# Nikhil-Kulkarni/RayTrace-miniapp

Hardware: AMD Instinct MI355X
Metric: ray_steps_per_sec (higher is better)
Workload: dtype f32+f64

## Files before the change

raytrace-miniapp_amd/csrc/rt_march.hip:

```cpp
#pragma once
#include "rt_math.h"

#include <cfloat>

namespace rt {

enum : int { ST_DONE_ESC = -2, ST_DONE = -1, ST_IDLE = 0, ST_STEP = 1, ST_XSETUP = 2, ST_CELL = 3, ST_ESC = 4 };
static_assert(ST_CELL + ST_DONE - ST_CELL == ST_DONE && ST_CELL + ST_DONE - ST_ESC == ST_DONE_ESC && ST_DONE_ESC < ST_IDLE &&
                  ST_DONE < ST_IDLE && ST_ESC > ST_CELL && ST_CELL > ST_XSETUP && ST_CELL > ST_STEP,
              "the order of the lane states");

typedef double f64x2 __attribute__((ext_vector_type(2)));
typedef float f32x4 __attribute__((ext_vector_type(4)));
typedef unsigned u32x4 __attribute__((ext_vector_type(4)));

__device__ __forceinline__ unsigned div_magic(unsigned x, unsigned mul, unsigned sh)
{
    return mul ? __umulhi(x, mul) >> sh : x;
}
__device__ __forceinline__ void grid_index(const DevRays &R, unsigned ridx, unsigned &i, unsigned &j, unsigned &k,
                                           unsigned &m)
{
    const unsigned ijkm = (unsigned) (R.first + (long long) ridx * R.stride);
    const unsigned q1   = div_magic(ijkm, R.div_mul[0], R.div_sh[0]);
    m                   = ijkm - q1 * (unsigned) R.ngb;
    const unsigned q2   = div_magic(q1, R.div_mul[1], R.div_sh[1]);
    k                   = q1 - q2 * (unsigned) R.nga;
    i                   = div_magic(q2, R.div_mul[2], R.div_sh[2]);
    j                   = q2 - i * (unsigned) R.ngy;
}

__device__ __forceinline__ void load_ray(const DevRays &R, unsigned ridx, rt_ray &ray, float &ta, float &tb,
                                         bool want_tan)
{
    if (R.list) {
        ray = R.list[ridx];
        if (want_tan) {
            ta = R.sxy[2 * (size_t) ridx];
            tb = R.sxy[2 * (size_t) ridx + 1];
        }
    } else {
        unsigned i, j, k, m;
        grid_index(R, ridx, i, j, k, m);
        ray.x      = (float) R.gx[i];
        ray.y      = (float) R.gy[j];
        ray.a      = (float) R.ga[k];
        ray.b      = (float) R.gb[m];
        if (want_tan) {
            ta = R.tan_a[k];
            tb = R.tan_b[m];
        }
    }
}

__device__ __attribute__((noinline)) float tan_wide(float x)
{
    if (!(fabsf(x) <= FLT_MAX))
        return x - x;
    return (float) tan((double) x);
}
__device__ __attribute__((noinline)) float atan_wide(float x)
{
    const float A0 = 3.3333334327e-01f, A1 = -2.0000000298e-01f, A2 = 1.4285714924e-01f, A3 = -1.1111110449e-01f,
                A4 = 9.0908870101e-02f, A5 = -7.6918758452e-02f, A6 = 6.6610731184e-02f, A7 = -5.8335702866e-02f,
                A8 = 4.9768779427e-02f, A9 = -3.6531571299e-02f, A10 = 1.6285819933e-02f;
    const unsigned hx = __float_as_uint(x), ix = hx & 0x7fffffffu;
    const bool neg = (hx >> 31) != 0u;
    if (ix >= 0x4c000000u) {
        if (ix > 0x7f800000u)
            return x + x;
        const float r = 1.5707962513e+00f + 7.5497894159e-08f;
        return neg ? -r : r;
    }
    float hi, lo;
    x = fabsf(x);
    if (ix < 0x3f980000u) {
        if (ix < 0x3f300000u) {
            hi = 4.6364760399e-01f;
            lo = 5.0121582440e-09f;
            x  = (2.0f * x - 1.0f) / (2.0f + x);
        } else {
            hi = 7.8539812565e-01f;
            lo = 3.7748947079e-08f;
            x  = (x - 1.0f) / (x + 1.0f);
        }
    } else {
        if (ix < 0x401c0000u) {
            hi = 9.8279368877e-01f;
            lo = 3.4473217170e-08f;
            x  = (x - 1.5f) / (1.0f + 1.5f * x);
        } else {
            hi = 1.5707962513e+00f;
            lo = 7.5497894159e-08f;
            x  = -1.0f / x;
        }
    }
    const float z = x * x, w = z * z;
    const float s1 = z * (A0 + w * (A2 + w * (A4 + w * (A6 + w * (A8 + w * A10)))));
    const float s2 = w * (A1 + w * (A3 + w * (A5 + w * (A7 + w * A9))));
    const float r  = hi - ((x * (s1 + s2) - lo) - x);
    return neg ? -r : r;
}

__device__ __attribute__((noinline)) float ktanf_flt32(float x, float y, int iy)
{
    const float T[13] = { 3.3333334327e-01f, 1.3333334029e-01f, 5.3968254477e-02f, 2.1869488060e-02f, 8.8632395491e-03f,
                          3.5920790397e-03f, 1.4562094584e-03f, 5.8804126456e-04f, 2.4646313977e-04f, 7.8179444245e-05f,
                          7.1407252108e-05f, -1.8558637748e-05f, 2.5907305826e-05f };
    const float pio4 = 7.8539812565e-01f, pio4lo = 3.7748947079e-08f;
    float z, r, v, w, s;
    const int hx = (int) __float_as_uint(x), ix = hx & 0x7fffffff;
    if (ix < 0x39000000) {
        if ((int) x == 0) {
            if ((ix | (iy + 1)) == 0)
                return 1.0f / fabsf(x);
            else if (iy == 1)
                return x;
            else
                return -1.0f / x;
        }
    }
    if (ix >= 0x3f2ca140) {
        if (hx < 0) {
            x = -x;
            y = -y;
        }
        z = pio4 - x;
        w = pio4lo - y;
        x = z + w;
        y = 0.0f;
        if (fabsf(x) < 0x1p-13f)
            return (1 - ((hx >> 30) & 2)) * iy * (1.0f - 2 * iy * x);
    }
    z = x * x;
    w = z * z;
    r = T[1] + w * (T[3] + w * (T[5] + w * (T[7] + w * (T[9] + w * T[11]))));
    v = z * (T[2] + w * (T[4] + w * (T[6] + w * (T[8] + w * (T[10] + w * T[12])))));
    s = z * x;
    r = y + z * (s * (r + v) + y);
    r += T[0] * s;
    w = x + r;
    if (ix >= 0x3f2ca140) {
        v = (float) iy;
        return (float) (1 - ((hx >> 30) & 2)) * (v - 2.0f * (x - (w * w / (w + v) - r)));
    }
    if (iy == 1)
        return w;
    float a, t;
    z = __uint_as_float(__float_as_uint(w) & 0xfffff000u);
    v = r - (z - x);
    t = a = -1.0f / w;
    t = __uint_as_float(__float_as_uint(t) & 0xfffff000u);
    s = 1.0f + t * z;
    return t + a * (s + t * v);
}
__device__ __attribute__((noinline)) float tanf_flt32_wide(float x)
{
    const float pio2_1 = 1.5707855225e+00f, pio2_1t = 1.0804334124e-05f, pio2_2 = 1.0804273188e-05f,
                pio2_2t = 6.0770999344e-11f;
    const int hx = (int) __float_as_uint(x), ix = hx & 0x7fffffff;
    if (ix <= 0x3f490fda)
        return ktanf_flt32(x, 0.0f, 1);
    float y0, y1, z;
    if (hx > 0) {
        z = x - pio2_1;
        if ((ix & 0xfffffff0) != 0x3fc90fd0) {
            y0 = z - pio2_1t;
            y1 = (z - y0) - pio2_1t;
        } else {
            z -= pio2_2;
            y0 = z - pio2_2t;
            y1 = (z - y0) - pio2_2t;
        }
    } else {
        z = x + pio2_1;
        if ((ix & 0xfffffff0) != 0x3fc90fd0) {
            y0 = z + pio2_1t;
            y1 = (z - y0) + pio2_1t;
        } else {
            z += pio2_2;
            y0 = z + pio2_2t;
            y1 = (z - y0) + pio2_2t;
        }
    }
    return ktanf_flt32(y0, y1, -1);
}

__device__ __forceinline__ float tanf_flt32_kernel(float x)
{
    const float ax = fabsf(x);
    if (ax < 0x1p-13f)
        return x;
    if (ax > 0.2f) {
        if (!(ax <= FLT_MAX))
            return x - x;
        return ax <= 1.375f ? tanf_flt32_wide(x) : tan_wide(x);
    }
    const float T0 = 3.3333334327e-01f, T1 = 1.3333334029e-01f, T2 = 5.3968254477e-02f, T3 = 2.1869488060e-02f,
                T4 = 8.8632395491e-03f, T5 = 3.5920790397e-03f, T6 = 1.4562094584e-03f, T7 = 5.8804126456e-04f,
                T8 = 2.4646313977e-04f, T9 = 7.8179444245e-05f, T10 = 7.1407252108e-05f, T11 = -1.8558637748e-05f,
                T12 = 2.5907305826e-05f;
    const float z = x * x;
    const float w = z * z;
    float r       = T1 + w * (T3 + w * (T5 + w * (T7 + w * (T9 + w * T11))));
    const float v = z * (T2 + w * (T4 + w * (T6 + w * (T8 + w * (T10 + w * T12)))));
    const float s = z * x;
    r             = 0.0f + z * (s * (r + v) + 0.0f);
    r += T0 * s;
    return x + r;
}

__device__ __forceinline__ float atanf_flt32_kernel(float x)
{
    const float ax = fabsf(x);
    if (ax < 0x1p-29f)
        return x;
    if (!(ax < 0.4375f))
        return atan_wide(x);
    const float A0 = 3.3333334327e-01f, A1 = -2.0000000298e-01f, A2 = 1.4285714924e-01f, A3 = -1.1111110449e-01f,
                A4 = 9.0908870101e-02f, A5 = -7.6918758452e-02f, A6 = 6.6610731184e-02f, A7 = -5.8335702866e-02f,
                A8 = 4.9768779427e-02f, A9 = -3.6531571299e-02f, A10 = 1.6285819933e-02f;
    const float z  = x * x;
    const float w  = z * z;
    const float s1 = z * (A0 + w * (A2 + w * (A4 + w * (A6 + w * (A8 + w * A10)))));
    const float s2 = w * (A1 + w * (A3 + w * (A5 + w * (A7 + w * A9))));
    return x - x * (s1 + s2);
}

extern "C" __global__ void __launch_bounds__(256) rt_seed_tab_kernel(const DevSeed sd, const DevRays R, double *sf,
                                                                     unsigned char *sin)
{
    const int n0 = R.ngx, n1 = R.ngy, n2 = R.nga, n3 = R.ngb;
    for (int t = (int) (blockIdx.x * blockDim.x + threadIdx.x); t < n0 + n1 + n2 + n3; t += (int) (gridDim.x * blockDim.x)) {
        int d           = t < n0 ? 0 : (t < n0 + n1 ? 1 : (t < n0 + n1 + n2 ? 2 : 3));
        const int i     = t - (d > 0 ? n0 : 0) - (d > 1 ? n1 : 0) - (d > 2 ? n2 : 0);
        const double *g = d == 0 ? R.gx : (d == 1 ? R.gy : (d == 2 ? R.ga : R.gb));
        const double v  = (double) (float) g[i];
        const bool in   = v >= sd.x[d][0] && v <= sd.x[d][sd.dim[d] - 1];
        sin[t]          = in ? 1 : 0;
        sf[t]           = in ? pchip_eval(sd.dim[d], sd.x[d], sd.f[d], v) : 0.0;
    }
}

__device__ __forceinline__ unsigned selftest_hash(unsigned x)
{
    x ^= x >> 16;
    x *= 0x7feb352du;
    x ^= x >> 15;
    x *= 0x846ca68bu;
    x ^= x >> 16;
    return x;
}
extern "C" __global__ void __launch_bounds__(256) rt_selftest_kernel(unsigned long long *counts)
{
    const unsigned lo = 0x3f700000u, hi = 0x3f880000u;
    const unsigned n_fast = hi - lo, n_other = 1u << 24;
    unsigned long long checked = 0, bad = 0;
    const unsigned long long tid = (unsigned long long) blockIdx.x * blockDim.x + threadIdx.x;
    const unsigned long long nth = (unsigned long long) gridDim.x * blockDim.x;
    for (unsigned long long t = tid; t < (unsigned long long) n_fast + n_other; t += nth) {
        const unsigned u = t < n_fast ? lo + (unsigned) t : (unsigned) (t - n_fast) << 8;
        float q          = __uint_as_float(u);
        const float a    = inv_norm(q);
        asm volatile("" : "+v"(q));
        const float b = 1.0f / sqrtf(q);
        checked++;
        if (__float_as_uint(a) != __float_as_uint(b) && !(a != a && b != b))
            bad++;
    }
    for (unsigned long long t = tid; t < (4ull << 23); t += nth) {
        float n       = __uint_as_float(0x3e800000u + (unsigned) t);
        const float a = fdiv_one_nr(n);
        asm volatile("" : "+v"(n));
        const float b = 1.0f / n;
        checked++;
        bad += __float_as_uint(a) != __float_as_uint(b) ? 1 : 0;
    }
    for (unsigned long long t = tid; t < (1ull << 28); t += nth) {
        const unsigned h0 = selftest_hash((unsigned) t * 2u + 1u), h1 = selftest_hash((unsigned) t * 2u + 0x9e3779b9u);
        const int ea = -84 + (int) (h0 % 84u), eb = -78 + (int) (h1 % 122u);
        if (ea - eb >= 96 || eb - ea >= 96 || ea - eb < -120)
            continue;
        float x = __uint_as_float(((unsigned) (ea + 127) << 23) | (selftest_hash(h0) & 0x7fffffu));
        float y = __uint_as_float(((unsigned) (eb + 127) << 23) | (selftest_hash(h1) & 0x7fffffu));
        const float a = fdiv_nr(x, y);
        asm volatile("" : "+v"(x), "+v"(y));
        const float b = x / y;
        checked++;
        bad += __float_as_uint(a) != __float_as_uint(b) ? 1 : 0;
    }
    if (tid == 0) {
        float inf = __uint_as_float(0x7f800000u), qnan = __uint_as_float(0x7fc00000u), big = 3.0e38f;
        asm volatile("" : "+v"(inf), "+v"(qnan), "+v"(big));
        const unsigned pio2 = 0x3fc90fdbu;
        const float t0 = tanf_flt32_kernel(inf), t1 = tanf_flt32_kernel(-inf), t2 = tanf_flt32_kernel(qnan), t3 = tan_wide(inf),
                    t4 = tan_wide(qnan), t5 = tanf_flt32_kernel(big);
        const float a0 = atanf_flt32_kernel(inf), a1 = atanf_flt32_kernel(-inf), a2 = atanf_flt32_kernel(qnan),
                    a3 = atanf_flt32_kernel(big), a4 = atanf_flt32_kernel(-big);
        checked += 11;
        bad += (t0 == t0) + (t1 == t1) + (t2 == t2) + (t3 == t3) + (t4 == t4) + (__float_as_uint(t5) == 0x7fc12345u);
        bad += (__float_as_uint(a0) != pio2) + (__float_as_uint(a1) != (pio2 | 0x80000000u)) + (a2 == a2) +
               (__float_as_uint(a3) != pio2) + (__float_as_uint(a4) != (pio2 | 0x80000000u));
    }
    atomicAdd(&counts[0], checked);
    atomicAdd(&counts[1], bad);
}

extern "C" __global__ void __launch_bounds__(256) rt_tan_kernel(const rt_ray *rays, unsigned long long n, float *sxy)
{
    unsigned long long i = (unsigned long long) blockIdx.x * blockDim.x + threadIdx.x;
    if (i < n) {
        rt_ray r       = rays[i];
        sxy[2 * i]     = tanf_flt32_kernel(1e-3f * r.a);
        sxy[2 * i + 1] = tanf_flt32_kernel(1e-3f * r.b);
    }
}

__device__ __forceinline__ int bisect_interval(const Interval *iv, int n, double v)
{
    int lo = 0, hi = n - 1;
    while (hi - lo != 1) {
        int mid = (hi + lo) / 2;
        if (iv[mid].hi >= v)
            hi = mid;
        else
            lo = mid;
    }
    return hi;
}
__device__ __forceinline__ int guess_interval(int n, float g0, float inv_h, float v)
{
    return (int) fminf(fmaxf((v - g0) * inv_h, 0.0f), (float) (n - 2)) + 1;
}

#ifdef RT_INSTRUMENT
__device__ unsigned long long g_inst[8];
__device__ unsigned long long g_prune[4];
__device__ unsigned short g_ray_iters[1u << 23];
#endif
#ifdef RT_TIMEBLOCKS
__device__ unsigned long long g_inst[8];
__device__ unsigned long long g_retire[4];
#endif
#ifdef RT_WAVETIMES
__device__ unsigned long long g_wt[8];
__device__ unsigned long long g_wt_end[8192], g_wt_dry[8192];
constexpr int WT_TRACE = 64;
__device__ unsigned long long g_wt_trace[8192][WT_TRACE];
__device__ unsigned g_wt_blocks[8192][WT_TRACE][6];
__device__ unsigned long long g_wt_pub[8192][4];
__device__ unsigned long long g_wt_vm[8192];
#endif
#if defined(RT_INSTRUMENT) || defined(RT_TIMEBLOCKS) || defined(RT_WAVETIMES)
struct MarchDiag {
    static __device__ __forceinline__ unsigned wave_number() { return blockIdx.x * (blockDim.x >> 6) + (threadIdx.x >> 6); }
    static __device__ __forceinline__ bool first_active_lane()
    {
        return (int) (threadIdx.x & 63) == __ffsll((long long) __ballot(1)) - 1;
    }
#ifdef RT_INSTRUMENT
    unsigned w[3] = { 0, 0, 0 }, a[3] = { 0, 0, 0 }, ray_iters = 0;
#endif
#if defined(RT_TIMEBLOCKS) || defined(RT_WAVEBLOCKS)
    unsigned long long tb_acc[6] = { 0, 0, 0, 0, 0, 0 }, tb_last = __builtin_readcyclecounter(), tb_iters = 0;
#endif
#ifdef RT_TIMEBLOCKS
    unsigned rt_fin = 0, rt_blk = 0, rt_refill = 0, rt_dry = 0;
#endif
#ifdef RT_WAVETIMES
    const unsigned long long wt_start = __builtin_amdgcn_s_memrealtime();
    unsigned long long wt_dry = 0, pub_t0 = 0;
    unsigned wt_a_runs = 0, wt_b_runs = 0, wave_iter = 0;
#endif
    __device__ __forceinline__ void tick(int i)
    {
#ifdef RT_INSTRUMENT
        a[i]++;
        w[i] += first_active_lane() ? 1u : 0u;
#endif
    }
    __device__ __forceinline__ void mark(int i)
    {
#if defined(RT_TIMEBLOCKS) || defined(RT_WAVEBLOCKS)
        const unsigned long long now = __builtin_readcyclecounter();
        tb_acc[i] += now - tb_last;
        tb_last = now;
#endif
    }
    __device__ __forceinline__ void iteration(int st, int lane, int n_idle)
    {
#ifdef RT_INSTRUMENT
        ray_iters += st > ST_IDLE ? 1u : 0u;
#endif
#ifdef RT_TIMEBLOCKS
        tb_iters++;
#endif
#ifdef RT_WAVETIMES
        if ((++wave_iter & 15u) == 0u) {
            const unsigned wid = wave_number(), smp = wave_iter >> 4;
            if (lane == 0 && wid < 8192u && smp < (unsigned) WT_TRACE) {
                g_wt_trace[wid][smp] = (__builtin_amdgcn_s_memrealtime() & 0xffffffffffull) | ((unsigned long long) (WAVE - n_idle) << 40) |
                                       ((unsigned long long) wt_a_runs << 48) | ((unsigned long long) wt_b_runs << 56);
                g_wt_trace[wid][0] = smp;
#ifdef RT_WAVEBLOCKS
                for (int b = 0; b < 6; b++)
                    g_wt_blocks[wid][smp][b] = (unsigned) tb_acc[b];
#endif
            }
#ifdef RT_WAVEBLOCKS
            for (int b = 0; b < 6; b++)
                tb_acc[b] = 0;
#endif
            wt_a_runs = wt_b_runs = 0;
        }
#endif
    }
    __device__ __forceinline__ void counters_dry()
    {
#ifdef RT_WAVETIMES
        wt_dry = __builtin_amdgcn_s_memrealtime();
#endif
    }
    __device__ __forceinline__ void blocks_run(bool a_runs, bool lane_wants_b)
    {
#ifdef RT_WAVETIMES
        wt_a_runs += a_runs ? 1u : 0u;
        wt_b_runs += __ballot(lane_wants_b) != 0ull ? 1u : 0u;
#endif
    }
    __device__ __forceinline__ void finishing(int st)
    {
#ifdef RT_TIMEBLOCKS
        rt_fin += (__ballot(st < ST_IDLE) != 0ull && first_active_lane()) ? 1u : 0u;
#endif
    }
    __device__ __forceinline__ void retire_block(int st, bool more)
    {
#ifdef RT_TIMEBLOCKS
        rt_blk += __ballot(st < ST_IDLE) != 0ull ? 1u : 0u;
        rt_dry += more ? 0u : 1u;
#endif
    }
    __device__ __forceinline__ void refill()
    {
#ifdef RT_TIMEBLOCKS
        rt_refill++;
#endif
    }
    __device__ __forceinline__ void ray_retired(unsigned ridx)
    {
#ifdef RT_INSTRUMENT
        if (ridx < (1u << 23))
            g_ray_iters[ridx] = (unsigned short) (ray_iters < 65535u ? ray_iters : 65535u);
        ray_iters = 0;
#endif
    }
    __device__ __forceinline__ void publish_begin()
    {
#ifdef RT_WAVETIMES
        pub_t0 = __builtin_amdgcn_s_memrealtime();
#endif
    }
    __device__ __forceinline__ void publish_stores_landed()
    {
#ifdef RT_WAVETIMES
        const unsigned long long now = __builtin_amdgcn_s_memrealtime();
        atomicAdd(&g_wt_vm[wave_number() & 8191u], now - pub_t0);
        pub_t0 = now;
#endif
    }
    __device__ __forceinline__ void publish_end()
    {
#ifdef RT_WAVETIMES
        const unsigned long long dt = __builtin_amdgcn_s_memrealtime() - pub_t0;
        unsigned long long *q       = g_wt_pub[wave_number() & 8191u];
        atomicAdd(&q[0], dt);
        atomicAdd(&q[1], 1ull);
        atomicMax(&q[3], dt);
#endif
    }
    static __device__ __forceinline__ void push_retry()
    {
#ifdef RT_WAVETIMES
        atomicAdd(&g_wt_pub[wave_number() & 8191u][2], 1ull);
#endif
    }
    __device__ __forceinline__ void tiny_dividend()
    {
#ifdef RT_INSTRUMENT
        if (first_active_lane())
            atomicAdd(&g_inst[6], 1ull);
#endif
    }
    __device__ __forceinline__ void prune(int i)
    {
#ifdef RT_INSTRUMENT
        if (first_active_lane())
            atomicAdd(&g_prune[i], 1ull);
#endif
    }
    __device__ __forceinline__ void wave_end(int lane)
    {
#ifdef RT_WAVETIMES
        if (lane == 0) {
            const unsigned long long wt_end = __builtin_amdgcn_s_memrealtime();
            atomicMin(&g_wt[0], wt_start);
            atomicMax(&g_wt[1], wt_start);
            const unsigned n = atomicAdd((unsigned *) &g_wt[6], 1u);
            if (n < 8192)
                g_wt_end[n] = wt_end | ((unsigned long long) (threadIdx.x >> 6) << 56), g_wt_dry[n] = wt_dry;
        }
#endif
#ifdef RT_TIMEBLOCKS
        const unsigned fin_wave = wave_sum_u32(rt_fin);
        if (lane == 0) {
            for (int i = 0; i < 6; i++)
                atomicAdd(&g_inst[i], tb_acc[i]);
            atomicAdd(&g_inst[7], tb_iters);
            atomicAdd(&g_retire[0], (unsigned long long) fin_wave);
            atomicAdd(&g_retire[1], (unsigned long long) rt_blk);
            atomicAdd(&g_retire[2], (unsigned long long) rt_refill);
            atomicAdd(&g_retire[3], (unsigned long long) rt_dry);
        }
#endif
#ifdef RT_INSTRUMENT
        for (int i = 0; i < 3; i++) {
            const unsigned tw = wave_sum_u32(w[i]), ta = wave_sum_u32(a[i]);
            if (lane == 0) {
                atomicAdd(&g_inst[2 * i], (unsigned long long) tw);
                atomicAdd(&g_inst[2 * i + 1], (unsigned long long) ta);
            }
        }
#endif
    }
};
#else
struct MarchDiag {
    __device__ __forceinline__ void tick(int) {}
    __device__ __forceinline__ void mark(int) {}
    __device__ __forceinline__ void iteration(int, int, int) {}
    __device__ __forceinline__ void counters_dry() {}
    __device__ __forceinline__ void blocks_run(bool, bool) {}
    __device__ __forceinline__ void finishing(int) {}
    __device__ __forceinline__ void retire_block(int, bool) {}
    __device__ __forceinline__ void refill() {}
    __device__ __forceinline__ void ray_retired(unsigned) {}
    __device__ __forceinline__ void publish_begin() {}
    __device__ __forceinline__ void publish_stores_landed() {}
    __device__ __forceinline__ void publish_end() {}
    static __device__ __forceinline__ void push_retry() {}
    __device__ __forceinline__ void tiny_dividend() {}
    __device__ __forceinline__ void prune(int) {}
    __device__ __forceinline__ void wave_end(int) {}
};
#endif

struct TileList {
    unsigned *head;
    unsigned *next;
    unsigned *lnode;
    unsigned *nalloc;
    unsigned cap;
    unsigned *rem;
    unsigned *marching;
    unsigned n_waves;
    unsigned split;
    unsigned k_part;
};
constexpr unsigned TILE_NONE = 0xffffffffu;
constexpr unsigned TILE_PART_FLAG = 1u << 30, TILE_PART_SHIFT = 28, TILE_ID_MASK = (1u << TILE_PART_SHIFT) - 1u;
__device__ __forceinline__ unsigned tile_node(unsigned entry)
{
    return (entry & TILE_ID_MASK) * 4u + ((entry & TILE_PART_FLAG) ? (entry >> TILE_PART_SHIFT) & 3u : 0u);
}
constexpr unsigned TILE_REF_GLOBAL = 1u << 31;
__device__ __forceinline__ void tile_push(const TileList &T, unsigned tile)
{
    const unsigned id = __hip_atomic_fetch_add(T.nalloc, 1u, __ATOMIC_RELAXED, __HIP_MEMORY_SCOPE_WORKGROUP);
    unsigned old      = __hip_atomic_load(T.head, __ATOMIC_RELAXED, __HIP_MEMORY_SCOPE_WORKGROUP);
    if (id < T.cap) {
        __hip_atomic_store(&T.lnode[2u * id], tile, __ATOMIC_RELAXED, __HIP_MEMORY_SCOPE_WORKGROUP);
        for (;;) {
            __hip_atomic_store(&T.lnode[2u * id + 1u], old, __ATOMIC_RELAXED, __HIP_MEMORY_SCOPE_WORKGROUP);
            asm volatile("s_waitcnt lgkmcnt(0)" ::: "memory");
            if (__hip_atomic_compare_exchange_strong(T.head, &old, id, __ATOMIC_RELAXED, __ATOMIC_RELAXED, __HIP_MEMORY_SCOPE_WORKGROUP))
                return;
            MarchDiag::push_retry();
        }
    }
    tile |= TILE_REF_GLOBAL;
    for (;;) {
        __hip_atomic_store(&T.next[tile_node(tile & ~TILE_REF_GLOBAL)], old, __ATOMIC_RELAXED, __HIP_MEMORY_SCOPE_WORKGROUP);
        asm volatile("s_waitcnt vmcnt(0)" ::: "memory");
        if (__hip_atomic_compare_exchange_strong(T.head, &old, tile, __ATOMIC_RELAXED, __ATOMIC_RELAXED, __HIP_MEMORY_SCOPE_WORKGROUP))
            return;
        MarchDiag::push_retry();
    }
}
__device__ __forceinline__ void tile_publish(const TileList &T, unsigned tile)
{
    bool parts = T.split == 2u;
    if (T.split == 1u)
        parts = __hip_atomic_load(T.head, __ATOMIC_RELAXED, __HIP_MEMORY_SCOPE_WORKGROUP) == TILE_NONE &&
                __hip_atomic_load(T.marching, __ATOMIC_RELAXED, __HIP_MEMORY_SCOPE_WORKGROUP) * 8u <= T.n_waves;
    if (parts && T.k_part != 0u) {
        for (unsigned q = 0; q < 4u; q++)
            tile_push(T, tile | (q << TILE_PART_SHIFT) | TILE_PART_FLAG);
    } else {
        tile_push(T, tile);
    }
}
__device__ __forceinline__ unsigned tile_pop(const TileList &T)
{
    unsigned old = __hip_atomic_load(T.head, __ATOMIC_RELAXED, __HIP_MEMORY_SCOPE_WORKGROUP);
    while (old != TILE_NONE) {
        const unsigned nxt = (old & TILE_REF_GLOBAL)
                                 ? __hip_atomic_load(&T.next[tile_node(old & ~TILE_REF_GLOBAL)], __ATOMIC_RELAXED, __HIP_MEMORY_SCOPE_WORKGROUP)
                                 : __hip_atomic_load(&T.lnode[2u * old + 1u], __ATOMIC_RELAXED, __HIP_MEMORY_SCOPE_WORKGROUP);
        if (__hip_atomic_compare_exchange_strong(T.head, &old, nxt, __ATOMIC_RELAXED, __ATOMIC_RELAXED, __HIP_MEMORY_SCOPE_WORKGROUP))
            break;
    }
    if (old == TILE_NONE)
        return TILE_NONE;
    return (old & TILE_REF_GLOBAL) ? (old & ~TILE_REF_GLOBAL) : __hip_atomic_load(&T.lnode[2u * old], __ATOMIC_RELAXED, __HIP_MEMORY_SCOPE_WORKGROUP);
}

template <bool LDS_TAB> __device__ __forceinline__ void march_load_tables(const DevParams &P, unsigned char *lds_raw)
{
    if (LDS_TAB) {
        const uint4 *src = reinterpret_cast<const uint4 *>(P.blob);
        uint4 *dst       = reinterpret_cast<uint4 *>(lds_raw);
        const unsigned n16 = P.blob_bytes / 16, step = blockDim.x;
        for (unsigned i0 = threadIdx.x; i0 < n16; i0 += 8 * step) {
            uint4 v[8];
#pragma unroll
            for (int u = 0; u < 8; u++) {
                const unsigned i = i0 + (unsigned) u * step;
                v[u]             = src[i < n16 ? i : i0];
            }
#pragma unroll
            for (int u = 0; u < 8; u++) {
                const unsigned i = i0 + (unsigned) u * step;
                if (i < n16)
                    dst[i] = v[u];
            }
        }
        __syncthreads();
    }
}

enum : int { MARCH_OPT_PRUNE = 1, MARCH_OPT_NO_NTEST = 2, MARCH_OPT_PRUNE_H24 = 4, MARCH_OPT_SCAN = 8 };
constexpr unsigned SCAN_BND_BYTES = 20u, SCAN_BND_ROW = WAVE * SCAN_BND_BYTES;
RT_HD inline size_t scan_bnd_off(unsigned ridx, int j, int L)
{
    return ((size_t) (ridx >> 6) * (size_t) (L - 1) + (size_t) (j - 1)) * SCAN_BND_ROW + (size_t) (ridx & 63u) * SCAN_BND_BYTES;
}
RT_HD inline size_t scan_bnd_bytes(unsigned long long n_rays, int L)
{
    return (size_t) ((n_rays + WAVE - 1) / WAVE) * (size_t) (L > 1 ? L - 1 : 0) * SCAN_BND_ROW;
}
__device__ __forceinline__ BlobGain march_blob_header(const BlobGain *hdr, int i, unsigned lds_base)
{
    BlobGain g = hdr[i];
    g.off_ix   = (int) ((unsigned) g.off_ix + lds_base);
    g.off_iy   = (int) ((unsigned) g.off_iy + lds_base);
    g.off_node = (int) ((unsigned) g.off_node + lds_base);
    return g;
}
template <bool LDS_TAB, bool BOUNDED, bool FUSED, int MODE = 0, int OPT = 0>
__device__ __forceinline__ void march_wave(const DevParams &P, unsigned char *lds_raw, const TileList done)
{
    const int lane        = lane_id();
    const int L           = P.L;
    const int S           = L * RT_N_SUB;
    const unsigned n_rays = P.ray_end;
    const bool backward   = MODE == 1 ? true : ((MODE == 2 || MODE == 3) ? false : P.method == 1);
    const bool use_emis   = MODE == 1 ? true : ((MODE == 2 || MODE == 4) ? false : P.use_emis != 0);
    const bool path_on    = MODE == 0 ? P.path_on != 0 : false;
    const unsigned CH     = P.chunk;
    constexpr int REFILL  = 8;

    const unsigned char *tab = LDS_TAB ? lds_raw : P.blob;
    const BlobGain *hdr = reinterpret_cast<const BlobGain *>(tab);
    const unsigned lds_base = LDS_TAB ? (unsigned) (size_t) (__attribute__((address_space(3))) unsigned char *) lds_raw : 0u;

    static_assert(RT_N_SUB == 3, "sub-segment ends are tabulated for three sub-segments");
    float zs0 = (P.dz0 * (0.0f + 1.0f) / RT_N_SUB), zs1 = (P.dz0 * (1.0f + 1.0f) / RT_N_SUB),
          zs2 = (P.dz0 * (2.0f + 1.0f) / RT_N_SUB);
    asm volatile("" : "+v"(zs0), "+v"(zs1), "+v"(zs2));

    unsigned chunk_next = 0, chunk_end = 0;
    unsigned fetched_end = 0, cur_slot = 0;
    unsigned cslot       = 0;
    bool more           = true;
    unsigned refill_at = (unsigned) REFILL;
    const unsigned n_launch_rays = n_rays - P.ray_begin;
    const unsigned n_chunks      = (n_launch_rays + CH - 1) / CH;
    unsigned shard = blockIdx.x & 7u, shards_seen_empty = 0;
    const unsigned n_main = n_chunks - (P.late_chunks < n_chunks ? P.late_chunks : 0u);
    const bool late_wave  = (unsigned) __builtin_amdgcn_readfirstlane((int) (threadIdx.x >> 6)) - P.late_first < P.late_waves;
    unsigned zone = 0;

    int st        = ST_IDLE;
    unsigned ridx = 0;
    int seg = 0, iz = 0, ii = 0;
    float z = 0.0f, z_stop = 0.0f;
    float z_lim = 0.0f;
    float px = 0, py = 0, pz = 0, sx = 0, sy = 0, sz = 1;
    float gacc = 0, eacc = 0;
    int cell_last = 0, sub = 0;
    unsigned char *recp = P.rec;
    unsigned lane12     = 0;
    BlobGain G    = march_blob_header(hdr, 1, lds_base);
    unsigned steps = 0;
    unsigned any_bits = 0;
    int c00 = 0;
    float f00 = 1, f10 = 1, f01 = 1, f11 = 1;
    double dnx0 = 0, dnx1 = 0, dny0 = 0, dny1 = 0;
    f64x2 ix0 = { 0.0, 1.0 }, iy0 = { 0.0, 1.0 };
    f32x4 ix1 = { 1.0f, 0.0f, 0.0f, 0.0f }, iy1 = { 1.0f, 0.0f, 0.0f, 0.0f };
    float g0 = 0, E0 = 0;
    float dzrem = 0, zc = 0, path = 0;
    float rx = 0, ry = 0, rz = 0, n = 0, n0 = 0, gxn = 0, gyn = 0, lim2 = 0, dzcap = 0, hsum = 0;
    unsigned tot_steps = 0, tot_esc = 0, tot_rays = 0, tot_skip = 0;
    unsigned spin = 0;
    MarchDiag diag;
    for (;;) {
        diag.mark(5);
        unsigned long long idle2      = __ballot(st <= ST_IDLE);
        const unsigned long long idle = idle2;
        int n_idle                    = (int) __popcll(idle);
        asm volatile("" : "+s"(n_idle));
        diag.iteration(st, lane, n_idle);
        if (!BOUNDED) {
            if (((++spin) & 0xfffu) == 0u && spin >= P.spin_limit) {
                spin = 0;
                if (st > ST_IDLE) {
                    sx = sy = sz = 0.0f;
                    st           = ST_ESC;
                }
            }
        }
        if ((unsigned) n_idle >= refill_at) {
            diag.mark(0);
            diag.retire_block(st, more);
            if (st < ST_IDLE) {
                const bool escaped = st == ST_DONE_ESC;
                unsigned fl        = F_VALID;
                if (escaped)
                    fl |= F_ESCAPED;
                if (use_emis && any_bits == 0u)
                    fl |= F_SKIP;
                RecMeta m;
                m.px          = px;
                m.py          = py;
                m.sx          = sx;
                m.sy          = sy;
                m.sz          = sz;
                m.flags_steps = fl | ((unsigned) sub << REC_NDONE_SHIFT) |
                                ((steps < 0xfffffu ? steps : 0xfffffu) << REC_STEPS_SHIFT);
                unsigned char *metap = recp + (int) REC_SLOT_ROW * (backward ? sub + 1 : S - sub) + lane12;
#ifndef RT_ABL_NOMETA
                *reinterpret_cast<RecMeta *>(metap) = m;
#else
                if (m.px == 1234.5f)
                    *reinterpret_cast<RecMeta *>(metap) = m;
#endif
                diag.ray_retired(ridx);
                tot_steps += steps;
                tot_esc += escaped ? 1u : 0u;
                tot_skip += (fl & F_SKIP) ? 1u : 0u;
                tot_rays++;
                st = ST_IDLE;
                if (FUSED) {
                    if (__hip_atomic_fetch_add(&done.rem[cslot], 0xffffffffu, __ATOMIC_RELAXED, __HIP_MEMORY_SCOPE_WAVEFRONT) == 1u) {
                        diag.publish_begin();
                        asm volatile("s_waitcnt vmcnt(0)" ::: "memory");
                        diag.publish_stores_landed();
                        tile_publish(done, ridx >> 6);
                        diag.publish_end();
                    }
                }
            }
            diag.mark(3);
            if (more) {
                diag.refill();
                const int rank = (int) __builtin_amdgcn_mbcnt_hi((unsigned) (idle >> 32),
                                                                 __builtin_amdgcn_mbcnt_lo((unsigned) idle, 0u));
                int need = n_idle, off = 0;
                bool got = false;
                while (need > 0) {
                    if (chunk_next == chunk_end && !(FUSED && chunk_next != fetched_end)) {
                        unsigned c = 0;
                        if (lane == 0)
                            c = atomicAdd(&P.ctl->next_tile[P.launch_id][shard][zone * 8u], 1u);
                        c = (unsigned) __builtin_amdgcn_readfirstlane((int) c) * 8u + shard + zone * n_main;
                        if (c >= (zone ? n_chunks : n_main)) {
                            if (++shards_seen_empty == 8) {
                                if (zone == 0u && late_wave && n_main < n_chunks) {
                                    zone              = 1u;
                                    shards_seen_empty = 0;
                                    continue;
                                }
                                more = false;
                                refill_at = 0u;
                                diag.counters_dry();
                                break;
                            }
                            shard = (shard + 1) & 7u;
                            continue;
                        }
                        chunk_next = P.ray_begin + c * CH;
                        chunk_end  = (n_rays - chunk_next < CH) ? n_rays : chunk_next + CH;
                        if (FUSED) {
                            fetched_end = chunk_end;
                            chunk_end   = chunk_next;
                        }
                    }
                    if (FUSED && chunk_next == chunk_end) {
                        const unsigned in_use    = lane < 32 ? __hip_atomic_load(&done.rem[lane], __ATOMIC_RELAXED, __HIP_MEMORY_SCOPE_WAVEFRONT) : 1u;
                        const unsigned slot_busy = ~(unsigned) __ballot(lane < 32 && in_use == 0u);
                        const int fs = __builtin_ffs((int) ~slot_busy) - 1;
                        if (fs < 0)
                            break;
                        chunk_end = fetched_end - chunk_next < (unsigned) WAVE ? fetched_end : chunk_next + (unsigned) WAVE;
                        cur_slot  = (unsigned) fs;
                        if (lane == 0)
                            __hip_atomic_store(&done.rem[fs], chunk_end - chunk_next, __ATOMIC_RELAXED, __HIP_MEMORY_SCOPE_WAVEFRONT);
                    }
                    int avail = (int) (chunk_end - chunk_next);
                    int take  = avail < need ? avail : need;
                    if (st == ST_IDLE && !got && rank >= off && rank < off + take) {
                        ridx = chunk_next + (unsigned) (rank - off);
                        got  = true;
                        if (FUSED)
                            cslot = cur_slot;
                    }
                    chunk_next += (unsigned) take;
                    need -= take;
                    off += take;
                }
                if (!BOUNDED && __ballot(got) != 0ull)
                    spin = 0;
                if (got) {
                    rt_ray ray;
                    float ta = 0, tb = 0;
                    load_ray(P.rays, ridx, ray, ta, tb, true);
                    px = ray.x;
                    py = ray.y;
                    pz = 0.0f;
                    sx = ta;
                    sy = tb;
                    sz = 1.0f;
                    if (backward) {
                        sx = -sx;
                        sy = -sy;
                        sz = -sz;
                    }
                    renormalise(sx, sy, sz);
                    const BlobGain G0 = march_blob_header(hdr, backward ? P.N - 1 : 1, lds_base);
                    const float dsum  = sx + sy + sz;
                    const bool wild   = ((px != px) | (py != py) | (dsum != dsum)) &
                                      !((px < G0.lo_x) | (px > G0.hi_x) | (py < G0.lo_y) | (py > G0.hi_y));
                    if (path_on) {
                        float *pp = P.path + (size_t) ridx * 3 * (size_t) (S + 1) + 3 * (size_t) (backward ? S : 0);
                        pp[0]     = px;
                        pp[1]     = py;
                    }
                    recp      = P.rec + rec_slot_off(ridx, backward ? S - 1 : 0, P.rec_stride);
                    lane12    = (ridx & 63u) * 12u;
                    seg       = 0;
                    iz        = 0;
                    ii        = backward ? P.N - 1 : 1;
                    G         = G0;
                    z         = 0.0f;
                    z_stop    = zs0;
                    z_lim     = 0.995f * zs0;
                    gacc      = 0.0f;
                    eacc      = 0.0f;
                    cell_last = 0;
                    steps     = 0;
                    sx        = wild ? 0.0f : sx;
                    sy        = wild ? 0.0f : sy;
                    sz        = wild ? 0.0f : sz;
                    any_bits  = P.no_skip;
                    sub       = 0;
                    st        = wild ? ST_ESC : ST_CELL;
                }
                idle2 = __ballot(st == ST_IDLE);
            }
        }
        if (idle2 == ~0ull) {
            if (!more)
                break;
        } else {

        diag.mark(0);
        const unsigned long long want_a = __ballot(st >= ST_CELL);
        int park_at = (int) P.park;
        if (!more || (int) P.park > 12 || REFILL > 8) {
            const int n_live = WAVE - (int) __popcll(idle2);
            const int fifth  = (n_live * 13 + 63) >> 6;
            park_at          = fifth < (int) P.park ? fifth : (int) P.park;
        }
        const bool do_a = (int) __popcll(want_a) >= park_at || (~(idle2 | want_a)) == 0ull;
        diag.blocks_run(do_a && want_a != 0ull, st == ST_XSETUP);
        if (do_a && st >= ST_CELL) {
            bool in_seg        = (st == ST_CELL) & (z < z_lim);
            if (!in_seg) {
#ifndef RT_ABL_NOSTORE
                *reinterpret_cast<RecSlot *>(recp) = RecSlot{ gacc, eacc, cell_last };
#endif
                recp += backward ? -(int) REC_SLOT_ROW : (int) REC_SLOT_ROW;
                any_bits |= (__float_as_uint(gacc) | __float_as_uint(eacc)) & 0x7fffffffu;
                if (path_on) {
                    float *pp = P.path + (size_t) ridx * 3 * (size_t) (S + 1);
                    for (int zz = iz; zz < (st == ST_ESC ? RT_N_SUB : iz + 1); zz++) {
                        const int idx = RT_N_SUB * (ii - 1) + (backward ? RT_N_SUB - zz - 1 : zz + 1);
                        pp[3 * idx]     = px;
                        pp[3 * idx + 1] = py;
                    }
                }
                gacc      = 0.0f;
                eacc      = 0.0f;
                cell_last = 0;
                sub++;
                const bool wrap = iz == RT_N_SUB - 1;
                const bool fin  = (st == ST_ESC) | (sub == S);
                iz              = wrap ? 0 : iz + 1;
                z               = wrap ? 0.0f : z;
                st              = fin ? ST_CELL + ST_DONE - st : ST_CELL;
                diag.finishing(st);
                if (wrap & !fin) {
                    if (OPT & MARCH_OPT_SCAN) {
                        unsigned char *bnd = reinterpret_cast<unsigned char *>(((unsigned long long) P.pad_march[1] << 32) | (unsigned long long) P.pad_march[0]);
                        float *q           = reinterpret_cast<float *>(bnd + scan_bnd_off(ridx, seg + 1, L));
                        q[0]               = px;
                        q[1]               = py;
                        q[2]               = sx;
                        q[3]               = sy;
                        q[4]               = sz;
                    }
                    seg++;
                    ii = backward ? P.N - seg - 1 : seg + 1;
                    G  = march_blob_header(hdr, ii, lds_base);
                }
                z_stop = iz == 0 ? zs0 : (iz == 1 ? zs1 : zs2);
                z_lim  = 0.995f * z_stop;
                in_seg = !fin & (z < z_lim);
            }
            diag.mark(1);
            if (in_seg) {
#include "rt_march_cell.inc"
            }
        }
        diag.mark(2);
        if (st == ST_XSETUP) {
#include "rt_march_xsetup.inc"
            lim2  = dzrem - zc;
            dzcap = P.c_cap * lim2;
            rx    = 0.0f;
            ry    = 0.0f;
            rz    = 0.0f;
            n     = n0;
            hsum  = 0.0f;
            st    = ST_STEP;
            diag.tick(1);
        }

        diag.mark(4);
        if (st == ST_STEP) {
            const float lim0 = 0.1f * ix1.x, lim1 = 0.1f * iy1.x;
            bool run;
            {
#include "rt_march_step.inc"
            }
            if (!run) {
                path += hsum;
                px += rx;
                py += ry;
                pz += rz;
                zc += fabsf(rz);
                const float ya = G.mirror_y != 0 ? fabsf(py) : py;
                if ((px > ix1.y) & (px < ix1.z) & (ya > iy1.y) & (ya < iy1.z) & ((double) zc < 0.999 * (double) dzrem)) {
                    st = ST_XSETUP;
                } else {
                    z += fabsf(pz);
                    gacc += g0 * path;
                    eacc += E0 * path;
                    cell_last = c00;
                    steps++;
                    diag.tick(2);
                    st = ST_CELL;
                }
            }
        }
        }
    }
    diag.wave_end(lane);
    {
        unsigned s = wave_sum_u32(tot_steps), e = wave_sum_u32(tot_esc);
        unsigned k = wave_sum_u32(tot_skip), r = wave_sum_u32(tot_rays);
        if (lane == 0) {
            atomicAdd(&P.ctl->cell_steps, (unsigned long long) s);
            atomicAdd(&P.ctl->n_escaped, (unsigned long long) e);
            atomicAdd(&P.ctl->n_skipped, (unsigned long long) k);
            atomicAdd(&P.ctl->n_rays, (unsigned long long) r);
        }
    }
}

template <bool LDS_TAB, bool BOUNDED, int MODE = 0, int OPT = 0>
__global__ void __launch_bounds__(LDS_TAB ? 1024 : 256) rt_march_kernel(const DevParams P)
{
    extern __shared__ __align__(16) unsigned char lds_raw[];
    march_load_tables<LDS_TAB>(P, lds_raw);
    march_wave<LDS_TAB, BOUNDED, false, MODE, OPT>(P, lds_raw, TileList{ nullptr, nullptr, nullptr, nullptr, 0u, nullptr, nullptr, 0u, 0u, 0u });
}

}
```

raytrace-miniapp_amd/csrc/rt_march_cell.inc:

```
                if ((px < G.lo_x) | (px > G.hi_x) | (py < G.lo_y) | (py > G.hi_y) | (sz * sz <= 0.01f)) {
                    st = ST_ESC;
                } else {
                    const Interval *ivx = reinterpret_cast<const Interval *>(tab + ((unsigned) G.off_ix - lds_base));
                    const Interval *ivy = reinterpret_cast<const Interval *>(tab + ((unsigned) G.off_iy - lds_base));
                    f64x2 tx, ty;
                    u32x4 q00, q10, q01, q11;
                    auto gather = [&](int k1, int k2, int c) {
                        const unsigned ox = __umul24((unsigned) k1, (unsigned) sizeof(Interval)) + (unsigned) G.off_ix;
                        const unsigned oy = __umul24((unsigned) k2, (unsigned) sizeof(Interval)) + (unsigned) G.off_iy;
                        static_assert(sizeof(Node) == 16, "node offsets are formed by a shift");
                        const unsigned oa = ((unsigned) c << 4) + (unsigned) G.off_node;
                        const unsigned ob = ((unsigned) G.Nx << 4) + oa;
                        if (LDS_TAB) {
                            asm volatile("ds_read_b128 %0, %10\n\t"
                                         "ds_read_b128 %1, %10 offset:16\n\t"
                                         "ds_read_b128 %2, %10 offset:32\n\t"
                                         "ds_read_b128 %3, %11\n\t"
                                         "ds_read_b128 %4, %11 offset:16\n\t"
                                         "ds_read_b128 %5, %11 offset:32\n\t"
                                         "ds_read_b128 %6, %12\n\t"
                                         "ds_read_b128 %7, %12 offset:16\n\t"
                                         "ds_read_b128 %8, %13\n\t"
                                         "ds_read_b128 %9, %13 offset:16\n\t"
                                         "s_waitcnt lgkmcnt(0)"
                                         : "=&v"(ix0), "=&v"(ix1), "=&v"(tx), "=&v"(iy0), "=&v"(iy1), "=&v"(ty), "=&v"(q00), "=&v"(q10),
                                           "=&v"(q01), "=&v"(q11)
                                         : "v"(ox), "v"(oy), "v"(oa), "v"(ob));
                        } else {
                            const unsigned char *t = tab;
                            ix0 = *reinterpret_cast<const f64x2 *>(t + ox);
                            ix1 = *reinterpret_cast<const f32x4 *>(t + ox + 16);
                            tx  = *reinterpret_cast<const f64x2 *>(t + ox + 32);
                            iy0 = *reinterpret_cast<const f64x2 *>(t + oy);
                            iy1 = *reinterpret_cast<const f32x4 *>(t + oy + 16);
                            ty  = *reinterpret_cast<const f64x2 *>(t + oy + 32);
                            q00 = *reinterpret_cast<const u32x4 *>(t + oa);
                            q10 = *reinterpret_cast<const u32x4 *>(t + oa + 16);
                            q01 = *reinterpret_cast<const u32x4 *>(t + ob);
                            q11 = *reinterpret_cast<const u32x4 *>(t + ob + 16);
                        }
                    };
                    auto node_n = [](const u32x4 &q) { return __hiloint2double((int) q.y, (int) q.x); };
                    const float ya      = G.mirror_y != 0 ? fabsf(py) : py;
                    const double pxd = (double) px, yad = (double) ya;
                    int k1     = guess_interval(G.Nx, G.x0f, G.inv_hxf, px);
                    int k2     = guess_interval(G.Ny, G.y0f, G.inv_hyf, ya);
                    c00        = (k1 - 1) + __mul24(k2 - 1, G.Nx);
                    gather(k1, k2, c00);
                    const bool ok = ((k1 == 1) | (ix0.x < pxd)) & ((k1 == G.Nx - 1) | (tx.x >= pxd)) &
                                    ((k2 == 1) | (iy0.x < yad)) & ((k2 == G.Ny - 1) | (ty.x >= yad));
                    if (!ok) {
                        k1  = bisect_interval(ivx, G.Nx, pxd);
                        k2  = bisect_interval(ivy, G.Ny, yad);
                        c00 = (k1 - 1) + __mul24(k2 - 1, G.Nx);
                        gather(k1, k2, c00);
                    }
                    const double n00 = node_n(q00), n10 = node_n(q10), n01 = node_n(q01), n11 = node_n(q11);
                    f00       = (float) n00;
                    f10       = (float) n10;
                    f01       = (float) n01;
                    f11       = (float) n11;
                    dnx0      = n10 - n00;
                    dnx1      = n11 - n01;
                    dny0      = n01 - n00;
                    dny1      = n11 - n10;
                    const float u = (float) div_by_recip_pos0(pxd - ix0.x, tx.x - ix0.x, tx.y);
                    const float v = (float) div_by_recip_pos0(yad - iy0.x, ty.x - iy0.x, ty.y);
                    g0            = lerp2(u, v, __uint_as_float(q00.z), __uint_as_float(q10.z), __uint_as_float(q01.z),
                                          __uint_as_float(q11.z));
                    E0            = 0.0f;
                    if (use_emis) {
                        E0 = lerp2(u, v, __uint_as_float(q00.w), __uint_as_float(q10.w), __uint_as_float(q01.w),
                                   __uint_as_float(q11.w));
                        E0 = E0 >= 0 ? E0 : 0.0f;
                    }
                    pz    = 0.0f;
                    zc    = 0.0f;
                    path  = 0.0f;
                    dzrem = z_stop - z;
                    if ((px > ix1.y) & (px < ix1.z) & (ya > iy1.y) & (ya < iy1.z) & (dzrem > 0.0f)) {
                        st = ST_XSETUP;
                    } else {
                        z += fabsf(pz);
                        gacc += g0 * path;
                        eacc += E0 * path;
                        cell_last = c00;
                        steps++;
                        diag.tick(2);
                    }
                }
```

Measured before the change: 31.40 billion.

## Move compute phase before refill in the wave loop and carry live-lane count

Reorders the persistent wave loop so the cell/xsetup/step work runs at the top of each iteration and the retire/refill ballot runs after it. The live-lane count is now carried from the previous iteration's refill ballot instead of being recomputed, and the 'more' flag is folded into refill_at being zero. The adaptive park threshold is precomputed as a wave-uniform mask, and the loop exit becomes a single scalar test. This is meant to cut ballots and scalar overhead per iteration and change the divergence and parking schedule. It shifts when parking decisions are made, which may alter how well lanes stay occupied.

```diff
diff --git a/raytrace-miniapp_amd/csrc/rt_march.hip b/raytrace-miniapp_amd/csrc/rt_march.hip
--- a/raytrace-miniapp_amd/csrc/rt_march.hip
+++ b/raytrace-miniapp_amd/csrc/rt_march.hip
@@ -692,8 +692,8 @@
     unsigned chunk_next = 0, chunk_end = 0;
     unsigned fetched_end = 0, cur_slot = 0;
     unsigned cslot       = 0;
-    bool more           = true;
     unsigned refill_at = (unsigned) REFILL;
+    const unsigned adaptive_at = (unsigned) __builtin_amdgcn_readfirstlane(((int) P.park > 12 || REFILL > 8) ? -1 : 0);
     const unsigned n_launch_rays = n_rays - P.ray_begin;
     const unsigned n_chunks      = (n_launch_rays + CH - 1) / CH;
     unsigned shard = blockIdx.x & 7u, shards_seen_empty = 0;
@@ -725,12 +725,120 @@
     unsigned tot_steps = 0, tot_esc = 0, tot_rays = 0, tot_skip = 0;
     unsigned spin = 0;
     MarchDiag diag;
+    int n_live = 0;
     for (;;) {
+        {
+        diag.mark(0);
+        const unsigned long long want_a = __ballot(st >= ST_CELL);
+        int n_want                      = (int) __popcll(want_a);
+        asm volatile("" : "+s"(n_want));
+        int park_at = (int) P.park;
+        if (refill_at <= adaptive_at) {
+            int fifth = (n_live * 13 + 63) >> 6;
+            asm volatile("" : "+s"(fifth));
+            park_at = fifth < (int) P.park ? fifth : (int) P.park;
+        }
+        const bool do_a = n_want >= (park_at < n_live ? park_at : n_live);
+        diag.blocks_run(do_a && want_a != 0ull, st == ST_XSETUP);
+        if (do_a) {
+        asm volatile("");
+        if (st >= ST_CELL) {
+            bool in_seg        = (st == ST_CELL) & (z < z_lim);
+            if (!in_seg) {
+#ifndef RT_ABL_NOSTORE
+                *reinterpret_cast<RecSlot *>(recp) = RecSlot{ gacc, eacc, cell_last };
+#endif
+                recp += backward ? -(int) REC_SLOT_ROW : (int) REC_SLOT_ROW;
+                any_bits |= (__float_as_uint(gacc) | __float_as_uint(eacc)) & 0x7fffffffu;
+                if (path_on) {
+                    float *pp = P.path + (size_t) ridx * 3 * (size_t) (S + 1);
+                    for (int zz = iz; zz < (st == ST_ESC ? RT_N_SUB : iz + 1); zz++) {
+                        const int idx = RT_N_SUB * (ii - 1) + (backward ? RT_N_SUB - zz - 1 : zz + 1);
+                        pp[3 * idx]     = px;
+                        pp[3 * idx + 1] = py;
+                    }
+                }
+                gacc      = 0.0f;
+                eacc      = 0.0f;
+                cell_last = 0;
+                sub++;
+                const bool wrap = iz == RT_N_SUB - 1;
+                const bool fin  = (st == ST_ESC) | (sub == S);
+                iz              = wrap ? 0 : iz + 1;
+                z               = wrap ? 0.0f : z;
+                st              = fin ? ST_CELL + ST_DONE - st : ST_CELL;
+                diag.finishing(st);
+                if (wrap & !fin) {
+                    if (OPT & MARCH_OPT_SCAN) {
+                        unsigned char *bnd = reinterpret_cast<unsigned char *>(((unsigned long long) P.pad_march[1] << 32) | (unsigned long long) P.pad_march[0]);
+                        float *q           = reinterpret_cast<float *>(bnd + scan_bnd_off(ridx, seg + 1, L));
+                        q[0]               = px;
+                        q[1]               = py;
+                        q[2]               = sx;
+                        q[3]               = sy;
+                        q[4]               = sz;
+                    }
+                    seg++;
+                    ii = backward ? P.N - seg - 1 : seg + 1;
+                    G  = march_blob_header(hdr, ii, lds_base);
+                }
+                z_stop = iz == 0 ? zs0 : (iz == 1 ? zs1 : zs2);
+                z_lim  = 0.995f * z_stop;
+                in_seg = !fin & (z < z_lim);
+            }
+            diag.mark(1);
+            if (in_seg) {
+#include "rt_march_cell.inc"
+            }
+        }
+        }
+        diag.mark(2);
+        if (st == ST_XSETUP) {
+#include "rt_march_xsetup.inc"
+            lim2  = dzrem - zc;
+            dzcap = P.c_cap * lim2;
+            rx    = 0.0f;
+            ry    = 0.0f;
+            rz    = 0.0f;
+            n     = n0;
+            hsum  = 0.0f;
+            st    = ST_STEP;
+            diag.tick(1);
+        }
+
+        diag.mark(4);
+        if (st == ST_STEP) {
+            const float lim0 = 0.1f * ix1.x, lim1 = 0.1f * iy1.x;
+            bool run;
+            {
+#include "rt_march_step.inc"
+            }
+            if (!run) {
+                path += hsum;
+                px += rx;
+                py += ry;
+                pz += rz;
+                zc += fabsf(rz);
+                const float ya = G.mirror_y != 0 ? fabsf(py) : py;
+                if ((px > ix1.y) & (px < ix1.z) & (ya > iy1.y) & (ya < iy1.z) & ((double) zc < 0.999 * (double) dzrem)) {
+                    st = ST_XSETUP;
+                } else {
+                    z += fabsf(pz);
+                    gacc += g0 * path;
+                    eacc += E0 * path;
+                    cell_last = c00;
+                    steps++;
+                    diag.tick(2);
+                    st = ST_CELL;
+                }
+            }
+        }
+        }
         diag.mark(5);
-        unsigned long long idle2      = __ballot(st <= ST_IDLE);
-        const unsigned long long idle = idle2;
+        const unsigned long long idle = __ballot(st <= ST_IDLE);
         int n_idle                    = (int) __popcll(idle);
         asm volatile("" : "+s"(n_idle));
+        int n_idle2 = n_idle;
         diag.iteration(st, lane, n_idle);
         if (!BOUNDED) {
             if (((++spin) & 0xfffu) == 0u && spin >= P.spin_limit) {
@@ -743,7 +851,7 @@
         }
         if ((unsigned) n_idle >= refill_at) {
             diag.mark(0);
-            diag.retire_block(st, more);
+            diag.retire_block(st, refill_at != 0u);
             if (st < ST_IDLE) {
                 const bool escaped = st == ST_DONE_ESC;
                 unsigned fl        = F_VALID;
@@ -783,7 +891,7 @@
                 }
             }
             diag.mark(3);
-            if (more) {
+            if (refill_at != 0u) {
                 diag.refill();
                 const int rank = (int) __builtin_amdgcn_mbcnt_hi((unsigned) (idle >> 32),
                                                                  __builtin_amdgcn_mbcnt_lo((unsigned) idle, 0u));
@@ -802,7 +910,6 @@
                                     shards_seen_empty = 0;
                                     continue;
                                 }
-                                more = false;
                                 refill_at = 0u;
                                 diag.counters_dry();
                                 break;
@@ -887,115 +994,13 @@
                     sub       = 0;
                     st        = wild ? ST_ESC : ST_CELL;
                 }
-                idle2 = __ballot(st == ST_IDLE);
+                n_idle2 = (int) __popcll(__ballot(st == ST_IDLE));
+                asm volatile("" : "+s"(n_idle2));
             }
         }
-        if (idle2 == ~0ull) {
-            if (!more)
-                break;
-        } else {
-
-        diag.mark(0);
-        const unsigned long long want_a = __ballot(st >= ST_CELL);
-        int park_at = (int) P.park;
-        if (!more || (int) P.park > 12 || REFILL > 8) {
-            const int n_live = WAVE - (int) __popcll(idle2);
-            const int fifth  = (n_live * 13 + 63) >> 6;
-            park_at          = fifth < (int) P.park ? fifth : (int) P.park;
-        }
-        const bool do_a = (int) __popcll(want_a) >= park_at || (~(idle2 | want_a)) == 0ull;
-        diag.blocks_run(do_a && want_a != 0ull, st == ST_XSETUP);
-        if (do_a && st >= ST_CELL) {
-            bool in_seg        = (st == ST_CELL) & (z < z_lim);
-            if (!in_seg) {
-#ifndef RT_ABL_NOSTORE
-                *reinterpret_cast<RecSlot *>(recp) = RecSlot{ gacc, eacc, cell_last };
-#endif
-                recp += backward ? -(int) REC_SLOT_ROW : (int) REC_SLOT_ROW;
-                any_bits |= (__float_as_uint(gacc) | __float_as_uint(eacc)) & 0x7fffffffu;
-                if (path_on) {
-                    float *pp = P.path + (size_t) ridx * 3 * (size_t) (S + 1);
-                    for (int zz = iz; zz < (st == ST_ESC ? RT_N_SUB : iz + 1); zz++) {
-                        const int idx = RT_N_SUB * (ii - 1) + (backward ? RT_N_SUB - zz - 1 : zz + 1);
-                        pp[3 * idx]     = px;
-                        pp[3 * idx + 1] = py;
-                    }
-                }
-                gacc      = 0.0f;
-                eacc      = 0.0f;
-                cell_last = 0;
-                sub++;
-                const bool wrap = iz == RT_N_SUB - 1;
-                const bool fin  = (st == ST_ESC) | (sub == S);
-                iz              = wrap ? 0 : iz + 1;
-                z               = wrap ? 0.0f : z;
-                st              = fin ? ST_CELL + ST_DONE - st : ST_CELL;
-                diag.finishing(st);
-                if (wrap & !fin) {
-                    if (OPT & MARCH_OPT_SCAN) {
-                        unsigned char *bnd = reinterpret_cast<unsigned char *>(((unsigned long long) P.pad_march[1] << 32) | (unsigned long long) P.pad_march[0]);
-                        float *q           = reinterpret_cast<float *>(bnd + scan_bnd_off(ridx, seg + 1, L));
-                        q[0]               = px;
-                        q[1]               = py;
-                        q[2]               = sx;
-                        q[3]               = sy;
-                        q[4]               = sz;
-                    }
-                    seg++;
-                    ii = backward ? P.N - seg - 1 : seg + 1;
-                    G  = march_blob_header(hdr, ii, lds_base);
-                }
-                z_stop = iz == 0 ? zs0 : (iz == 1 ? zs1 : zs2);
-                z_lim  = 0.995f * z_stop;
-                in_seg = !fin & (z < z_lim);
-            }
-            diag.mark(1);
-            if (in_seg) {
-#include "rt_march_cell.inc"
-            }
-        }
-        diag.mark(2);
-        if (st == ST_XSETUP) {
-#include "rt_march_xsetup.inc"
-            lim2  = dzrem - zc;
-            dzcap = P.c_cap * lim2;
-            rx    = 0.0f;
-            ry    = 0.0f;
-            rz    = 0.0f;
-            n     = n0;
-            hsum  = 0.0f;
-            st    = ST_STEP;
-            diag.tick(1);
-        }
-
-        diag.mark(4);
-        if (st == ST_STEP) {
-            const float lim0 = 0.1f * ix1.x, lim1 = 0.1f * iy1.x;
-            bool run;
-            {
-#include "rt_march_step.inc"
-            }
-            if (!run) {
-                path += hsum;
-                px += rx;
-                py += ry;
-                pz += rz;
-                zc += fabsf(rz);
-                const float ya = G.mirror_y != 0 ? fabsf(py) : py;
-                if ((px > ix1.y) & (px < ix1.z) & (ya > iy1.y) & (ya < iy1.z) & ((double) zc < 0.999 * (double) dzrem)) {
-                    st = ST_XSETUP;
-                } else {
-                    z += fabsf(pz);
-                    gacc += g0 * path;
-                    eacc += E0 * path;
-                    cell_last = c00;
-                    steps++;
-                    diag.tick(2);
-                    st = ST_CELL;
-                }
-            }
-        }
-        }
+        n_live = WAVE - n_idle2;
+        if (((unsigned) n_live | refill_at) == 0u)
+            break;
     }
     diag.wave_end(lane);
     {
diff --git a/raytrace-miniapp_amd/csrc/rt_march_cell.inc b/raytrace-miniapp_amd/csrc/rt_march_cell.inc
--- a/raytrace-miniapp_amd/csrc/rt_march_cell.inc
+++ b/raytrace-miniapp_amd/csrc/rt_march_cell.inc
@@ -81,6 +81,7 @@
                     if ((px > ix1.y) & (px < ix1.z) & (ya > iy1.y) & (ya < iy1.z) & (dzrem > 0.0f)) {
                         st = ST_XSETUP;
                     } else {
+                        asm volatile("");
                         z += fabsf(pz);
                         gacc += g0 * path;
                         eacc += E0 * path;
```

After: 31.73 billion (median of 6 runs). 1.01x the previous value.
